# mahfuzalhasan/WaveFormer

Measured on AMD Instinct MI355X. Metric: 128³×4 volumes/sec fwd (1/2/4/8 MI355X) + Dice Δ vs reference, higher is better.
Workload: dtype bf16x3; 1 GPU; MultiscaleTransformer (WaveFormer encoder) forward, 128^3x4 crops; global_batch=8, per_gpu_batch=8, precision=bf16x3, parallelism=replicas x1 (no data-path collective), hip_graph=True

## Files before the change

include/waveformer_hip.h:

```cpp
#ifndef WAVEFORMER_HIP_H
#define WAVEFORMER_HIP_H

#include <stdint.h>

#ifdef __cplusplus
extern "C" {
#endif

#define WF_ABI_VERSION 26

enum { WF_PREC_BF16 = 0, WF_PREC_BF16X3 = 1, WF_PREC_FP16 = 2 };

enum {
  WF_OK = 0,
  WF_E_SHAPE = -1,
  WF_E_NULLPTR = -2,
  WF_E_LAUNCH = -3
};

int wf_abi_version(void);
const char* wf_last_error(void);


int wf_cast_f32_to_bf16(const float* in, uint16_t* out, int64_t n, void* stream);

int wf_split_f32_to_bf16x2(const float* in, uint16_t* out, int64_t n, void* stream);

int wf_split_f32_to_bf16x2_multi(const int64_t* table_dev, int64_t n, int64_t total,
                                 void* stream);

int wf_cast_f32_to_f16x2(const float* in, uint16_t* out, int64_t n, void* stream);
int wf_cast_f32_to_f16x2_multi(const int64_t* table_dev, int64_t n, int64_t total,
                               void* stream);

int wf_debug_poison_lds(int64_t blocks, int lds_bytes, void* stream);

int wf_patch_embed_fwd(const float* x, const float* w, const float* bias, float* out,
                       int64_t B, int64_t Cin, int64_t Cout, int64_t D, int64_t H, int64_t W,
                       void* stream);
int wf_patch_embed_ll_fwd(const float* x, const float* w, const float* bias, float* out,
                          const float* ln_w, const float* ln_b, float ln_eps, float* ll,
                          int64_t B, int64_t Cin, int64_t Cout, int64_t D, int64_t H, int64_t W,
// ... 165 lines not shown
                                        int64_t B, int64_t C, int64_t heads, float scale,
                                        int precision, void* stream, int qkv_mode);
int wf_window_attention_levels_fused(const int64_t* dhw, int nlev, int64_t B, int64_t C,
                                     int64_t heads, int precision);

int wf_msfuse_fwd(const float* const* src, const int64_t* src_dhw, int nsrc,
                  const float* shortcut, const float* branch_scale, float* out, float* stats,
                  float ln_eps, int64_t B, int64_t C, int64_t D, int64_t H, int64_t W,
                  void* stream);

int64_t wf_ccf_ffn_workspace_bytes(int64_t B, int64_t C, int64_t hidden, int64_t D, int64_t H,
                                   int64_t W, int precision);
int wf_ccf_ffn_fwd(const float* xh, const float* stats, const float* n2_w, const float* n2_b,
                   const uint16_t* pw_bf16x2, const float* pw_b, const float* ln1_w,
                   const float* ln1_b, float eps1, const float* dw_w, const float* dw_b,
                   const float* ln2_w, const float* ln2_b, float eps2,
                   const uint16_t* fc_bf16x2, const float* fc_b, const float* branch_scale,
                   float* out, void* workspace,
                   int64_t B, int64_t C, int64_t hidden, int64_t D, int64_t H, int64_t W,
                   int precision, void* stream);
int wf_ccf_ffn_stage(int stage, const float* xh, const float* stats, const float* n2_w,
                     const float* n2_b, const uint16_t* pw_bf16x2, const float* pw_b,
                     const float* ln1_w, const float* ln1_b, float eps1, const float* dw_w,
                     const float* dw_b, const float* ln2_w, const float* ln2_b, float eps2,
                     const uint16_t* fc_bf16x2, const float* fc_b, const float* branch_scale,
                     float* out, void* workspace, int64_t B, int64_t C, int64_t hidden,
                     int64_t D, int64_t H, int64_t W, int precision, void* stream);
int wf_ccf_ffn_plan(int64_t B, int64_t C, int64_t hidden, int64_t D, int64_t H, int64_t W,
                    int precision, int train, int64_t* offsets);

int wf_patch_merging_fwd(const float* x, const float* ln_w, const float* ln_b, float eps,
                         const uint16_t* red_bf16x2, int v2, float* out, int64_t B, int64_t C,
                         int64_t D, int64_t H, int64_t W, int precision, void* stream);

int wf_proj_out_fwd(const float* x, float* out, int normalize, float eps, int64_t B,
                    int64_t C, int64_t S, void* stream);
int wf_proj_out_cl_fwd(const float* x, float* out, float eps, int64_t M, int64_t C, void* stream);

int wf_importance_map(int mode, const float* sigma_scale, float* out, int64_t rd, int64_t rh,
                      int64_t rw, void* stream);

int wf_sliding_window_stitch(const float* patches, int64_t world, int64_t slots_per_round,
                             const float* importance_map, const int64_t* starts,
                             const int64_t* nwin, float* out, int64_t B, int64_t C, int64_t D,
                             int64_t H, int64_t W, int64_t rd, int64_t rh, int64_t rw,
                             void* stream);

int wf_sliding_window_stitch_partial(const float* patches, int64_t world, int64_t rank,
                                     const float* importance_map, const int64_t* starts,
                                     const int64_t* nwin, float* out, int64_t B, int64_t C,
                                     int64_t D, int64_t H, int64_t W, int64_t rd, int64_t rh,
                                     int64_t rw, void* stream);
int wf_sliding_window_normalize(const float* num, float* out, int64_t B, int64_t C, int64_t D,
                                int64_t H, int64_t W, void* stream);

int wf_tta_merge(const float* pred, const int* flips, int npass, float* out, int64_t C,
                 int64_t D, int64_t H, int64_t W, void* stream);


int wf_window_attention_fwd_train(const float* x, const float* ln_w, const float* ln_b,
                                  float ln_eps, const uint16_t* wqkv_bf16x2, const float* bqkv,
                                  const float* bias, const uint16_t* wproj_bf16x2,
                                  const float* bproj, float* out, void* workspace, float* lse,
                                  int64_t B, int64_t C, int64_t D1, int64_t H1, int64_t W1,
                                  int64_t ws, int64_t heads, float scale, int precision,
                                  void* stream);
// ... 144 lines not shown
```

waveformer_amd/_lib.py:

```python
from __future__ import annotations

import ctypes
import os
import threading

_HERE = os.path.dirname(os.path.abspath(__file__))
LIB_PATH = os.environ.get("WAVEFORMER_HIP_LIB", os.path.join(_HERE, "libwaveformer_hip.so"))

_P = ctypes.c_void_p
_I64 = ctypes.c_int64
_I = ctypes.c_int
_F = ctypes.c_float

SIGNATURES = {
    "wf_abi_version": (_I, []),
    "wf_last_error": (ctypes.c_char_p, []),
    "wf_cast_f32_to_bf16": (_I, [_P, _P, _I64, _P]),
    "wf_split_f32_to_bf16x2": (_I, [_P, _P, _I64, _P]),
    "wf_split_f32_to_bf16x2_multi": (_I, [_P, _I64, _I64, _P]),
    "wf_cast_f32_to_f16x2": (_I, [_P, _P, _I64, _P]),
    "wf_cast_f32_to_f16x2_multi": (_I, [_P, _I64, _I64, _P]),
    "wf_debug_poison_lds": (_I, [_I64, _I, _P]),
    "wf_patch_embed_ll_fwd": (_I, [_P, _P, _P, _P, _P, _P, _F, _P, _I64, _I64, _I64, _I64, _I64,
                                   _I64, _P]),
# ... 42 lines not shown
                                _I64, _I64, _I64, _F, _P, _P]),
    "wf_hf_refine_workspace_bytes": (_I64, [_I64, _I64]),
    "wf_hf_refine_fwd": (_I, [_P, _I64, _P, _P, _P, _P, _F, _P, _P, _I, _P, _P, _I64, _I64,
                              _I64, _I64, _I64, _P]),
    "wf_hf_refine_bwd_workspace_bytes": (_I64, [_I64] * 5),
    "wf_hf_refine_bwd": (_I, [_P, _I64, _P, _P, _P, _P, _F, _P, _P, _I, _P, _P, _P, _P, _P, _P,
                              _P, _P, _P, _P, _I64, _I64, _I64, _I64, _I64, _P]),
    "wf_norm_act_cl": (_I, [_P, _I64, _P, _P, _I64, _P, _P, _I64, _I64, _I64, _I64, _F, _P]),
    "wf_upsample_trilinear_cl": (_I, [_P, _P, _I64, _I64, _I64, _I64, _I64, _I64, _I64, _I64,
                                      _I, _P]),
    "wf_linear_fwd": (_I, [_P, _P, _P, _P, _I64, _I64, _I64, _I, _I, _P]),
    "wf_window_attention_fwd_table": (_I, [_P, _P, _P, _F, _P, _P, _P, _P, _P, _P, _P,
                                           _I64, _I64, _I64, _I64, _I64, _I64, _I64, _F, _I,
                                           _P]),
    "wf_rel_pos_bias": (_I, [_P, _P, _P, _I64, _I64, _I64, _P]),
    "wf_window_attention_workspace_bytes": (_I64, [_I64, _I64, _I64, _I64, _I64, _I]),
    "wf_window_attention_fwd": (_I, [_P, _P, _P, _F, _P, _P, _P, _P, _P, _P, _P,
                                     _I64, _I64, _I64, _I64, _I64, _I64, _I64, _F, _I, _P]),
    "wf_window_attention_levels_workspace_bytes": (_I64, [_P, _I, _I64, _I64, _I]),
    "wf_window_attention_fwd_levels": (_I, [_P, _P, _I, _P, _P, _P, _P, _P, _P, _P, _I64, _I64,
                                            _I64, _F, _I, _P]),
    "wf_window_attention_fwd_levels_mode": (_I, [_P, _P, _I, _P, _P, _P, _P, _P, _P, _P, _I64,
                                                 _I64, _I64, _F, _I, _P, _I]),
    "wf_window_attention_levels_fused": (_I, [_P, _I, _I64, _I64, _I64, _I]),
    "wf_msfuse_fwd": (_I, [_P, _P, _I, _P, _P, _P, _P, _F, _I64, _I64, _I64, _I64, _I64, _P]),
    "wf_ccf_ffn_workspace_bytes": (_I64, [_I64, _I64, _I64, _I64, _I64, _I64, _I]),
    "wf_ccf_ffn_fwd": (_I, [_P, _P, _P, _P, _P, _P, _P, _P, _F, _P, _P, _P, _P, _F, _P, _P,
                            _P, _P, _P, _I64, _I64, _I64, _I64, _I64, _I64, _I, _P]),
    "wf_ccf_ffn_stage": (_I, [_I, _P, _P, _P, _P, _P, _P, _P, _P, _F, _P, _P, _P, _P, _F, _P,
                              _P, _P, _P, _P, _I64, _I64, _I64, _I64, _I64, _I64, _I, _P]),
    "wf_ccf_ffn_plan": (_I, [_I64, _I64, _I64, _I64, _I64, _I64, _I, _I, _P]),
    "wf_patch_merging_fwd": (_I, [_P, _P, _P, _F, _P, _I, _P, _I64, _I64, _I64, _I64, _I64,
                                  _I, _P]),
    "wf_proj_out_fwd": (_I, [_P, _P, _I, _F, _I64, _I64, _I64, _P]),
    "wf_proj_out_cl_fwd": (_I, [_P, _P, _F, _I64, _I64, _P]),
    "wf_upsample_dwconv3d_stats_cl": (_I, [_P, _P, _P, _P, _P] + [_I64] * 8 + [_I, _P]),
    "wf_importance_map": (_I, [_I, _P, _P, _I64, _I64, _I64, _P]),
    "wf_sliding_window_stitch": (_I, [_P, _I64, _I64, _P, _P, _P, _P, _I64, _I64, _I64, _I64,
                                      _I64, _I64, _I64, _I64, _P]),
    "wf_tta_merge": (_I, [_P, _P, _I, _P, _I64, _I64, _I64, _I64, _P]),
    "wf_sliding_window_stitch_partial": (_I, [_P, _I64, _I64, _P, _P, _P, _P, _I64, _I64,
                                              _I64, _I64, _I64, _I64, _I64, _I64, _P]),
    "wf_sliding_window_normalize": (_I, [_P, _P, _I64, _I64, _I64, _I64, _I64, _P]),
    "wf_window_attention_fwd_train": (_I, [_P, _P, _P, _F, _P, _P, _P, _P, _P, _P, _P, _P,
                                           _I64, _I64, _I64, _I64, _I64, _I64, _I64, _F, _I,
                                           _P]),
    "wf_window_attention_bwd_workspace_bytes": (_I64, [_I64, _I64, _I64, _I64, _I64, _I64,
                                                       _I64]),
    "wf_window_attention_bwd_core": (_I, [_P, _P, _P, _P, _P, _P, _P, _P, _I64, _I64, _I64,
                                          _I64, _I64, _I64, _I64, _F, _P]),
    "wf_rel_pos_bias_bwd": (_I, [_P, _P, _P, _P, _I64, _I64, _I64, _P]),
    "wf_gemm_tn_workspace_bytes": (_I64, [_I64, _I64, _I64]),
    "wf_gemm_tn": (_I, [_P, _I64, _P, _I64, _P, _I64, _I, _P, _I64, _I64, _I64, _P]),
    "wf_colsum_parts": (_I64, [_I64]),
    "wf_colsum": (_I, [_P, _I64, _I64, _P, _I64, _P, _P, _P]),
    "wf_ln_act_fwd": (_I, [_P, _P, _P, _F, _I, _P, _I64, _I64, _P]),
    "wf_ln_bwd_workspace_floats": (_I64, [_I64, _I64]),
    "wf_ln_act_bwd": (_I, [_P, _P, _P, _F, _I, _P, _P, _P, _P, _P, _P, _I64, _I64, _P]),
    "wf_dwt3d_haar_bwd": (_I, [_P, _P, _P, _I64, _I64, _I64, _I64, _I64, _P]),
    "wf_haar_analysis_ncdhw": (_I, [_P, _I64, _I64, _P, _P, _P, _I64, _I64, _I64, _I64, _I64,
                                    _P]),
    "wf_interp_adjoint_axis": (_I, [_P, _P, _I64, _I64, _I64, _I64, _P, _I64, _P]),
    "wf_interp_adjoint_axis_ac": (_I, [_P, _P, _I64, _I64, _I64, _I64, _P]),
    "wf_dwconv3d_cl": (_I, [_P, _P, _P, _I, _P, _I64, _I64, _I64, _I64, _I64, _P]),
    "wf_dwconv_wgrad_ws_floats": (_I64, [_I64] * 5),
    "wf_dwconv3d_wgrad": (_I, [_P, _P, _P, _P, _I64, _I64, _I64, _I64, _I64, _P]),
    "wf_patch_merging_gather": (_I, [_P, _I, _P, _I64, _I64, _I64, _I64, _I64, _P]),
    "wf_patch_merging_scatter": (_I, [_P, _I, _P, _I64, _I64, _I64, _I64, _I64, _P]),
    "wf_patchify": (_I, [_P, _P, _I, _I64, _I64, _I64, _I64, _I64, _P]),
    "wf_transpose_cs": (_I, [_P, _P, _I64, _I64, _I64, _P]),
    "wf_region_masks": (_I, [_P, _I, _I64, _P, _I64, _P, _P, _P, _I64, _I64, _I64, _P]),
    "wf_overlap_counts": (_I, [_P, _P, _I64, _I64, _I64, _I64, _P, _P]),
    "wf_surface_edt_workspace_bytes": (_I64, [_I64, _I64, _I64, _I64]),
    "wf_surface_edt_sq": (_I, [_P, _I64, _I64, _I64, _I64, _P, _P, _P, _I64, _P]),
    "wf_surface_hist": (_I, [_P, _P, _P, _P, _I64, _I64, _I64, _I64, _P, _P]),
    "wf_hist_order_stats": (_I, [_P, _I64, _I64, _I64, _I64, _I64, _P, _I64, _P, _P]),
    "wf_nonzero_mask": (_I, [_P, _I64, _I64, _I64, _I64, _P, _P]),
    "wf_fill_holes_workspace_bytes": (_I64, [_I64, _I64, _I64]),
    "wf_fill_holes": (_I, [_P, _I64, _I64, _I64, _P, _P, _P, _I64, _P, _P]),
    "wf_box_moments_workspace_bytes": (_I64, [_I64, _I64, _I64, _I64]),
    "wf_box_moments": (_I, [_P, _I64, _I64, _I64, _I64, _P, _P, _P, _I64, _P]),
    "wf_crop_normalize": (_I, [_P, _I64, _I64, _I64, _I64, _P, _P, _P, _P]),
    "wf_crop_seg": (_I, [_P, _P, _I64, _I64, _I64, _P, _I, _P, _P, _P]),
    "wf_select_workspace_bytes": (_I64, [_I64]),
    "wf_select_scan": (_I, [_P, _I64, _I, _I, _P, _I64, _P, _P]),
    "wf_select_pick": (_I, [_P, _I64, _I64, _I64, _I, _I, _P, _I64, _P, _I64, _P, _P, _P, _P]),
    "wf_spline_prefilter_axis": (_I, [_P, _P, _I64, _I64, _I64, _I64, _I, _I, _P]),
    "wf_gauss_blur_axis": (_I, [_P, _P, _I64, _I64, _I64, _I64, _I, _P, _I, _P]),
    "wf_affine_sample": (_I, [_P, _P, _P] + [_I64] * 7 + [_P, _P, _P]),
    "wf_zoom_nearest": (_I, [_P] + [_I64] * 7 + [_P, _P]),
    "wf_zoom_cubic": (_I, [_P] + [_I64] * 7 + [_P, _P]),
    "wf_augment_pointwise_workspace_bytes": (_I64, [_I64, _I64]),
    "wf_augment_pointwise": (_I, [_P, _I64, _I64, _I, _P, _P, _P, _P, _P, _I64, _P]),
    "wf_channel_stats": (_I, [_P, _I64, _I64, _P, _P, _I64, _P]),
}

ABI_VERSION = 26
_lock = threading.Lock()
_lib = None
_err = None


class LibraryMissing(RuntimeError):
    pass


def load(path: str | None = None):
    global _lib, _err
    with _lock:
        if _lib is not None:
            return _lib
        p = path or LIB_PATH
        if not os.path.exists(p):
            _err = f"{p} not found: build it with `python -c 'import __graft_entry__ as g; g.build()'`"
            raise LibraryMissing(_err)
        lib = ctypes.CDLL(p)
        for name, (res, args) in SIGNATURES.items():
            fn = getattr(lib, name)
            fn.restype = res
            fn.argtypes = args
        ver = lib.wf_abi_version()
        if ver != ABI_VERSION:
            raise LibraryMissing(f"{p}: ABI version {ver}, expected {ABI_VERSION} (rebuild)")
        _lib = lib
        return _lib


def call(name: str, *args) -> None:
    lib = load()
    rc = getattr(lib, name)(*args)
# ... 8 lines not shown
```

waveformer_amd/csrc/ffn.hip:

```cpp
#include "kernels.hpp"

namespace wf {

template <typename T>
struct Store4;
template <>
struct Store4<uint16_t> {
  typedef bf16x4 vec;
  static __device__ __forceinline__ f32x4 up(vec u) {
    return f32x4{bf2f((uint16_t)u[0]), bf2f((uint16_t)u[1]), bf2f((uint16_t)u[2]),
                 bf2f((uint16_t)u[3])};
  }
  static __device__ __forceinline__ uint16_t down(float v) { return f2bf(v); }
  static __device__ __forceinline__ vec zero() { return vec{0, 0, 0, 0}; }
  static __device__ __forceinline__ void store4(uint16_t* p, f32x4 v) {
    bf16x4 o;
    o[0] = (short)f2bf(v.x);
    o[1] = (short)f2bf(v.y);
    o[2] = (short)f2bf(v.z);
    o[3] = (short)f2bf(v.w);
    *reinterpret_cast<bf16x4*>(p) = o;
  }
};
template <>
// ... 668 lines not shown
  if (run_dw) {
    if (ln2_loader)
      rc = launch_dwconv3d(h1, dw_w, dw_b, h2, ln2_pst, (int)B, (int)hidden, (int)D, (int)H, (int)W,
                           precision, s, nullptr,
                           plan.front == FFN_FRONT_PARTIALS ? ln1_st : nullptr, ln1_w, ln1_b);
    else
      rc = launch_dwconv_ln_gelu(h1, dw_w, dw_b, ln2_w, ln2_b, eps2, h2, (int)B, (int)hidden,
                                 (int)D, (int)H, (int)W, precision, s);
  }
  if (rc || !run_fc) return rc;
  GemmArgs f = fc_gemm_args(h2, ln2_loader ? ln2_pst : nullptr, ln2_w, ln2_b, eps2, fc_bf16x2, fc_b,
                            xh, stats, n2_w, n2_b, branch_scale, out, M, C, hidden, D * H * W,
                            precision);
  if (!train) {
    f.kpart = reinterpret_cast<float*>(h1);
    f.kpart_bytes = ws.h2 - ws.h1;
  }
  return launch_gemm(f, s, "wf_ccf_ffn_fwd(fc)");
}

extern "C" int wf_ccf_ffn_fwd(const float* xh, const float* stats, const float* n2_w,
                              const float* n2_b, const uint16_t* pw_bf16x2, const float* pw_b,
                              const float* ln1_w, const float* ln1_b, float eps1,
                              const float* dw_w, const float* dw_b, const float* ln2_w,
                              const float* ln2_b, float eps2, const uint16_t* fc_bf16x2,
                              const float* fc_b, const float* branch_scale, float* out,
                              void* workspace, int64_t B, int64_t C, int64_t hidden, int64_t D,
                              int64_t H, int64_t W, int precision, void* stream) {
  return wf_ccf_ffn_stage(0, xh, stats, n2_w, n2_b, pw_bf16x2, pw_b, ln1_w, ln1_b, eps1, dw_w,
                          dw_b, ln2_w, ln2_b, eps2, fc_bf16x2, fc_b, branch_scale, out,
                          workspace, B, C, hidden, D, H, W, precision, stream);
}

extern "C" int wf_patch_merging_fwd(const float* x, const float* ln_w, const float* ln_b,
                                    float eps, const uint16_t* red_bf16x2, int v2, float* out,
                                    int64_t B, int64_t C, int64_t D, int64_t H, int64_t W,
                                    int precision, void* stream) {
  WF_REQUIRE(B >= 1 && C % 8 == 0 && C >= 8, "C must be a positive multiple of 8");
  WF_REQUIRE(D % 2 == 0 && H % 2 == 0 && W % 2 == 0 && D >= 2 && H >= 2 && W >= 2,
             "odd sizes (the F.pad branch, wave_helper.py:180-182) are not supported");
  WF_REQUIRE(valid_prec(precision), "unknown precision");
  WF_REQUIRE_PTR(x);
  WF_REQUIRE_PTR(ln_w);
  WF_REQUIRE_PTR(ln_b);
  WF_REQUIRE_PTR(red_bf16x2);
  WF_REQUIRE_PTR(out);
  GemmArgs g{};
  g.prec = precision;
  g.a_src = x;
  g.a_bf16 = 0;
  g.a_C = (int)C;
  g.a_nseg = 8;
  g.a_map = MAP_MERGE;
  g.merge_code = v2 ? 0x76543210 : 0x71251240;
  g.mB = (int)B;
  g.mD = (int)D;
  g.mH = (int)H;
  g.mW = (int)W;
  g.a_ln = LN_COMPUTE;
  g.a_ln_w = ln_w;
  g.a_ln_b = ln_b;
  g.a_eps = eps;
  g.w = red_bf16x2;
  g.M = B * (D / 2) * (H / 2) * (W / 2);
  g.N = (int)(2 * C);
  g.K = (int)(8 * C);
  g.epi = EPI_STORE;
  g.bias = nullptr;
  g.out = out;
  g.out_bf16 = 0;
  g.ldo = 2 * C;
  if (try_launch_merge_resident(g, (hipStream_t)stream)) return check_launch("wf_patch_merging_fwd");
  return launch_gemm(g, (hipStream_t)stream, "wf_patch_merging_fwd");
}
```

waveformer_amd/csrc/kernels.hpp:

```cpp
#pragma once
#include "ffn_plan.hpp"
#include "wf_common.hpp"

namespace wf {

enum Prec { PREC_BF16 = 0, PREC_SPLIT = 1, PREC_FP16 = 2 };

typedef _Float16 f16x4 __attribute__((ext_vector_type(4)));
typedef _Float16 f16x8 __attribute__((ext_vector_type(8)));
__device__ __forceinline__ uint16_t f2h(float f) { return __builtin_bit_cast(uint16_t, (_Float16)f); }

template <int P>
__device__ __forceinline__ uint16_t op_cvt(float x) {
  if constexpr (P == PREC_FP16) return f2h(x);
  else return f2bf(x);
}
template <int P>
__device__ __forceinline__ short op_lo(float x, uint16_t hi) {
  if constexpr (P == PREC_SPLIT) return (short)f2bf(x - bf2f(hi));
  else return (short)0;
}
template <int P>
__device__ __forceinline__ f32x4 mma32(bf16x8 a, bf16x8 b, f32x4 c) {
  if constexpr (P == PREC_FP16)
    return __builtin_amdgcn_mfma_f32_16x16x32_f16(__builtin_bit_cast(f16x8, a),
                                                  __builtin_bit_cast(f16x8, b), c, 0, 0, 0);
  else return __builtin_amdgcn_mfma_f32_16x16x32_bf16(a, b, c, 0, 0, 0);
}
template <int P>
__device__ __forceinline__ f32x4 mma16(bf16x4 a, bf16x4 b, f32x4 c) {
  if constexpr (P == PREC_FP16)
    return __builtin_amdgcn_mfma_f32_16x16x16f16(__builtin_bit_cast(f16x4, a),
                                                 __builtin_bit_cast(f16x4, b), c, 0, 0, 0);
  else return __builtin_amdgcn_mfma_f32_16x16x16bf16_1k(a, b, c, 0, 0, 0);
// ... 82 lines not shown
  const float* r_scale;
  int64_t rows_per_sample;
  float* o_pstats;
  float* kpart;
  int64_t kpart_bytes;
  int ksplit;
  const float* lv_src[WF_MAX_LEVELS];
  int lv_row0[WF_MAX_LEVELS];
  int lv_D[WF_MAX_LEVELS], lv_H[WF_MAX_LEVELS], lv_W[WF_MAX_LEVELS];
};

int launch_gemm(const GemmArgs& g, hipStream_t s, const char* who);
int gemm_kc_pick_nt(const GemmArgs& g);
int launch_instnorm_partial(const float* x, int64_t ldx, int64_t B, int64_t C, int64_t P,
                            double* acc, hipStream_t s);
int try_launch_gemm_rows(const GemmArgs& g, hipStream_t s, bool single_chunk_only);

int launch_attn_core(const void* qkv, const float* bias, void* out, float* lse, int64_t Bw,
                     int N, int heads, int hd, float scale, int prec, hipStream_t s,
                     int table_ws = 0, int64_t pair_windows = -1, const GemmArgs* fused = nullptr);
bool attn_tbl_pair_loop(int64_t wh);

int launch_dwconv_ln_gelu(const void* in, const float* w, const float* b, const float* ln_w,
                          const float* ln_b, float eps, void* out, int B, int Hd, int D, int H,
                          int W, int prec, hipStream_t s);
int launch_dwconv3d(const void* in, const float* w, const float* b, void* out, float* pstats,
                    int B, int Hd, int D, int H, int W, int prec, hipStream_t s,
                    double* cstats = nullptr, const float* ln1_stats = nullptr,
                    const float* ln1_w = nullptr, const float* ln1_b = nullptr, int flip = 0);
int launch_ln_stats_finalize(const float* pstats, int np, int group, float eps, float* out,
                             int64_t M, hipStream_t s);
int try_launch_gemm_kc(const GemmArgs& g, hipStream_t s);
int try_launch_merge_resident(const GemmArgs& g, hipStream_t s);
int try_launch_pw2_resident(const GemmArgs& g, hipStream_t s);
int try_launch_gemm_lnw(const GemmArgs& g, hipStream_t s);
inline bool gemm_lnw_wide_shape(const GemmArgs& g) { return gemm_lnw_wide_shape(g.N, g.K); }

}

#include "ffn_dwfc_common.hpp"
```

waveformer_amd/csrc/merge.hip:

```cpp
#include <algorithm>

#include "gemm_common.hpp"

namespace wf {

constexpr int MR_C = 48;
constexpr int MR_K = 8 * MR_C;
constexpr int MR_N = 2 * MR_C;
constexpr int MR_NT = MR_N / 16;
constexpr int MR_KS = MR_K / 32;
constexpr int MR_KP = MR_K + WF_LDS_KPAD;
constexpr int MR_WAVES = 8;

template <int P>
__global__ __launch_bounds__(64 * MR_WAVES, 1) void merge_res_kernel(GemmArgs g) {
  constexpr bool SPLIT = P == PREC_SPLIT;
  constexpr int NPL = SPLIT ? 2 : 1;
  extern __shared__ __attribute__((aligned(16))) uint16_t Wl[];
  float* lnw = reinterpret_cast<float*>(Wl + NPL * MR_N * MR_KP);
  float* lnb = lnw + MR_K;
  const int tid = threadIdx.x, lane = tid & 63, wid = tid >> 6;
  const int l15 = lane & 15, g4 = lane >> 4;

  constexpr int OCT = MR_K / 8;
// ... 60 lines not shown
    const float rstd = rsqrtf(fmaxf(q / kf - ms * ms, 0.f) + g.a_eps);

    uint32_t wb = (uint32_t)((l15 * MR_KP + 8 * g4) * 2), lb = (uint32_t)(8 * g4 * 4);
    asm volatile("" : "+v"(wb), "+v"(lb));
    const char* Wb = reinterpret_cast<const char*>(Wl) + wb;
    const char* Lw = reinterpret_cast<const char*>(lnw) + lb;
    const char* Lb = reinterpret_cast<const char*>(lnb) + lb;
    f32x4 acc[MR_NT];
#pragma unroll
    for (int t = 0; t < MR_NT; ++t) acc[t] = f32x4{0.f, 0.f, 0.f, 0.f};
#pragma unroll
    for (int ks = 0; ks < MR_KS; ++ks) {
      __builtin_amdgcn_sched_barrier(0);
      bf16x8 ah, al;
      a_fragment<P>(a[ks], mean, rstd, reinterpret_cast<const float*>(Lw),
                    reinterpret_cast<const float*>(Lb), ks * 32, true, true, false, ah, al);
#pragma unroll
      for (int t = 0; t < MR_NT; ++t) {
        const int wo = (t * 16 * MR_KP + ks * 32) * 2;
        const bf16x8 bh = *reinterpret_cast<const bf16x8*>(Wb + wo);
        const bf16x8 bl = SPLIT ? *reinterpret_cast<const bf16x8*>(Wb + MR_N * MR_KP * 2 + wo) : bh;
        acc[t] = mma3<P>(acc[t], bh, bl, ah, al);
        if (t % 3 == 2) __builtin_amdgcn_sched_barrier(0);
      }
    }
    if (row < M) {
      float* o = reinterpret_cast<float*>(g.out) + (int64_t)row * g.ldo + 4 * g4;
#pragma unroll
      for (int t = 0; t < MR_NT; ++t) *reinterpret_cast<f32x4*>(o + 16 * t) = acc[t];
    }
  }
}

int try_launch_merge_resident(const GemmArgs& g, hipStream_t s) {
  static const bool off = getenv("WF_MERGE_RES") != nullptr && getenv("WF_MERGE_RES")[0] == '0';
  if (off || g.a_map != MAP_MERGE || g.a_C != MR_C || g.K != MR_K || g.N != MR_N ||
      g.a_ln != LN_COMPUTE || g.a_bf16 || g.out_bf16 || g.epi != EPI_STORE || g.bias ||
      g.o_pstats || g.ldo < MR_N || (g.prec != PREC_SPLIT && g.prec != PREC_FP16) || g.M < 1 ||
      g.M >= ((int64_t)1 << 31) - 16)
    return 0;
  const bool split = g.prec == PREC_SPLIT;
  const size_t lds = (size_t)(split ? 2 : 1) * MR_N * MR_KP * 2 + (size_t)2 * MR_K * 4;
  void (*kern)(GemmArgs) = split ? merge_res_kernel<PREC_SPLIT> : merge_res_kernel<PREC_FP16>;
  set_max_lds(reinterpret_cast<const void*>(kern), (int)lds);
  const int64_t ntiles = (g.M + 15) / 16;
  const unsigned gx = (unsigned)std::min<int64_t>(cdiv(ntiles, MR_WAVES), 256);
  hipLaunchKernelGGL(kern, dim3(gx), dim3(64 * MR_WAVES), lds, s, g);
  return 1;
}

}
```

waveformer_amd/network_models/wave_helper.py:

```python
from __future__ import annotations

import math
import threading
from typing import Optional, Tuple

import torch
import torch.nn as nn
import torch.nn.functional as F

from .. import autograd as wfa
from .. import library
from .. import ops
from .attention import Attention

_OPS = torch.ops.waveformer


def _conv_fan_out_init(m: nn.Module) -> None:
    if isinstance(m, (nn.Conv2d, nn.Conv3d)):
        fan_out = math.prod(m.kernel_size) * m.out_channels // m.groups
        m.weight.data.normal_(0, math.sqrt(2.0 / fan_out))
        if m.bias is not None:
            m.bias.data.zero_()

# ... 138 lines not shown
        return y.flatten(2).transpose(1, 2)


class PatchMergingV2(nn.Module):

    def __init__(self, dim: int, norm_layer=nn.LayerNorm, spatial_dims: int = 3) -> None:
        super().__init__()
        self.dim = dim
        if spatial_dims == 3:
            self.reduction = nn.Linear(8 * dim, 2 * dim, bias=False)
            self.norm = norm_layer(8 * dim)
        elif spatial_dims == 2:
            self.reduction = nn.Linear(4 * dim, 2 * dim, bias=False)
            self.norm = norm_layer(4 * dim)
        self._v2 = True

    def _merge_2d(self, x):
        b, h, w, c = x.shape
        if h % 2 or w % 2:
            x = F.pad(x, (0, 0, 0, w % 2, 0, h % 2))
        x = torch.cat([x[:, j::2, i::2, :] for i in range(2) for j in range(2)], -1)
        return self.reduction(self.norm(x))

    def forward(self, x):
        if x.dim() == 4:
            return self._merge_2d(x)
        if x.dim() != 5:
            raise ValueError(f"expecting 5D x, got {tuple(x.shape)}.")
        b, d, h, w, c = x.shape
        if d % 2 or h % 2 or w % 2:
            x = F.pad(x, (0, 0, 0, w % 2, 0, h % 2, 0, d % 2))
        x = x.contiguous()
        prec = wfa.prec_for(x, *self.parameters())
        return _OPS.patch_merging(x, self.norm.weight, self.norm.bias, float(self.norm.eps),
                                  self.reduction.weight, self._v2, prec)

    def _wf_split_params(self):
        return [self.reduction.weight]


class PatchMerging(PatchMergingV2):

    def __init__(self, dim: int, norm_layer=nn.LayerNorm, spatial_dims: int = 3) -> None:
        super().__init__(dim, norm_layer, spatial_dims)
        self._v2 = False


class CCF_FFN(nn.Module):

    def __init__(self, in_features, hidden_features=None, out_features=None,
                 act_layer=nn.GELU, norm_layer=nn.LayerNorm, drop=0., img_size=(48, 48, 48)):
        super().__init__()
        self.D, self.H, self.W = img_size[0], img_size[1], img_size[2]
        out_features = out_features or in_features
        hidden_features = hidden_features or in_features
        self.C_hid = hidden_features
        self.pwconv = nn.Conv3d(in_features, hidden_features, 1, 1, 0, bias=True)
        self.dwconv = nn.Conv3d(hidden_features, hidden_features, 3, 1, 1, bias=True,
                                groups=hidden_features)
        self.fc = nn.Linear(hidden_features, in_features)
        self.act = act_layer()
        self.norm1 = norm_layer(hidden_features)
        self.norm2 = norm_layer(hidden_features)
        if not (isinstance(self.act, nn.GELU) and self.act.approximate == "none"):
            raise NotImplementedError("CCF_FFN: only nn.GELU() (erf) is implemented")
        self.apply(self._init_weights)

    def _init_weights(self, m):
# ... 292 lines not shown
```

waveformer_amd/ops.py:

```python
from __future__ import annotations

import ctypes
import math
import os
import threading
import weakref
from typing import Dict, List, Optional, Sequence, Tuple

import torch

from . import _lib

DETAIL_KEYS = ("aad", "ada", "add", "daa", "dad", "dda", "ddd")


def _stream() -> int:
    return torch.cuda.current_stream().cuda_stream


def _ptr(t: Optional[torch.Tensor]) -> Optional[int]:
    return None if t is None else t.data_ptr()


def _check(t: torch.Tensor, name: str, dtype=torch.float32, contiguous=True) -> None:
# ... 1308 lines not shown
    fc = split_weight(fcw, prec=prec)
    out = torch.empty_like(xh)
    wsb = _lib.query("wf_ccf_ffn_workspace_bytes", B, C, hid, D, H, W, prec)
    work = torch.empty(wsb, dtype=torch.uint8, device=xh.device)
    args = (xh.data_ptr(), _ptr(stats), _ptr(n2w), _ptr(n2b),
            pw.data_ptr(), _ptr(pwb), l1w.data_ptr(), l1b.data_ptr(), float(eps1),
            dww.data_ptr(), dwb.data_ptr(), l2w.data_ptr(), l2b.data_ptr(), float(eps2),
            fc.data_ptr(), _ptr(fcb), _ptr(branch_scale),
            out.data_ptr(), work.data_ptr(), B, C, hid, D, H, W, prec, _stream())
    ccf_ffn_pwconv(args)
    ccf_ffn_dwconv(args, B * D * H * W, hid)
    ccf_ffn_fc(args)
    return out


def ccf_ffn_pwconv(args):
    _lib.call("wf_ccf_ffn_stage", 1, *args)


def ccf_ffn_dwconv(args, positions: int, hidden: int):
    _lib.call("wf_ccf_ffn_stage", 2, *args)


def ccf_ffn_fc(args):
    _lib.call("wf_ccf_ffn_stage", 3, *args)


def patch_merging(x_cl: torch.Tensor, norm: torch.nn.LayerNorm, reduction: torch.nn.Linear,
                  v2: bool = False) -> torch.Tensor:
    return _patch_merging_raw(x_cl, norm.weight, norm.bias, float(norm.eps), reduction.weight,
                              v2, _prec())


def _patch_merging_raw(x_cl, ln_w, ln_b, eps, red_w, v2, prec) -> torch.Tensor:
    _check(x_cl, "x")
    B, D, H, W, C = x_cl.shape
    red = split_weight(red_w, prec=prec)
    out = torch.empty((B, D // 2, H // 2, W // 2, 2 * C), dtype=torch.float32, device=x_cl.device)
    _lib.call("wf_patch_merging_fwd", x_cl.data_ptr(), ln_w.data_ptr(), ln_b.data_ptr(),
              float(eps), red.data_ptr(), int(bool(v2)), out.data_ptr(), B, C, D, H, W, prec,
              _stream())
    return out


BLEND_MODES = {"constant": 0, "gaussian": 1}


def importance_map(roi: Sequence[int], mode: str = "constant",
                   sigma_scale: Sequence[float] = (0.125, 0.125, 0.125),
                   device: Optional[torch.device] = None) -> torch.Tensor:
    if mode not in BLEND_MODES:
        raise ValueError(f"Unsupported mode: {mode}, available options are {sorted(BLEND_MODES)}.")
    rd, rh, rw = (int(v) for v in roi)
    device = torch.device(device) if device is not None else torch.device(
        "cuda", torch.cuda.current_device())
    if device.type != "cuda":
        raise RuntimeError("importance_map: GPU only")
    out = torch.empty((rd, rh, rw), dtype=torch.float32, device=device)
    sig = (ctypes.c_float * 3)(*[float(s) for s in sigma_scale])
    _lib.call("wf_importance_map", BLEND_MODES[mode], sig, out.data_ptr(), rd, rh, rw, _stream())
    return out


def sliding_window_stitch(patches: torch.Tensor, weight_map: torch.Tensor,
                          starts: Sequence[Sequence[int]], image_size: Sequence[int],
                          batch: int, world: int = 1, slots_per_round: int = 1) -> torch.Tensor:
    _check(patches, "patches")
    _check(weight_map, "importance_map")
    rows, C = patches.shape[:2]
    roi = tuple(patches.shape[2:])
    if tuple(weight_map.shape) != roi:
        raise ValueError(f"sliding_window_stitch: map {tuple(weight_map.shape)} != roi {roi}")
    nwin = [len(s) for s in starts]
    total = batch * nwin[0] * nwin[1] * nwin[2]
# ... 536 lines not shown
```

Baseline: 1317 volumes/s.

## Add persistent streaming patch-merging kernel with fused LayerNorm for C=96/192

Adds a persistent, register-streamed patch-merge kernel for C=96 and C=192 at inference. Each block loops over row tiles, gathers the 2x2x2 neighbours into LDS, computes LayerNorm there and runs the bf16x3 or fp16 MFMA GEMM. Weights are pre-permuted into a workspace so each wave streams its own slice through a triple-buffered register pipeline, and C=96 adds dedicated loader waves to prefetch the next tile. The aim is to replace the generic GEMM path for these merges. The cost is an extra weight-permute launch per call and a per-call workspace allocation.

```diff
diff --git a/include/waveformer_hip.h b/include/waveformer_hip.h
--- a/include/waveformer_hip.h
+++ b/include/waveformer_hip.h
@@ -7,7 +7,7 @@
 extern "C" {
 #endif
 
-#define WF_ABI_VERSION 26
+#define WF_ABI_VERSION 27
 
 enum { WF_PREC_BF16 = 0, WF_PREC_BF16X3 = 1, WF_PREC_FP16 = 2 };
 
@@ -239,6 +239,13 @@
 int wf_patch_merging_fwd(const float* x, const float* ln_w, const float* ln_b, float eps,
                          const uint16_t* red_bf16x2, int v2, float* out, int64_t B, int64_t C,
                          int64_t D, int64_t H, int64_t W, int precision, void* stream);
+int64_t wf_patch_merging_workspace_bytes(int64_t C, int precision);
+int wf_patch_merging_fwd_ws(const float* x, const float* ln_w, const float* ln_b, float eps,
+                            const uint16_t* red_bf16x2, int v2, float* out, int64_t B, int64_t C,
+                            int64_t D, int64_t H, int64_t W, int precision, int train,
+                            void* workspace, int64_t workspace_bytes, void* stream);
+int wf_patch_merging_plan(int64_t B, int64_t C, int64_t D, int64_t H, int64_t W, int precision,
+                          int train, int64_t* info);
 
 int wf_proj_out_fwd(const float* x, float* out, int normalize, float eps, int64_t B,
                     int64_t C, int64_t S, void* stream);
diff --git a/waveformer_amd/_lib.py b/waveformer_amd/_lib.py
--- a/waveformer_amd/_lib.py
+++ b/waveformer_amd/_lib.py
@@ -98,6 +98,10 @@
     "wf_ccf_ffn_plan": (_I, [_I64, _I64, _I64, _I64, _I64, _I64, _I, _I, _P]),
     "wf_patch_merging_fwd": (_I, [_P, _P, _P, _F, _P, _I, _P, _I64, _I64, _I64, _I64, _I64,
                                   _I, _P]),
+    "wf_patch_merging_workspace_bytes": (_I64, [_I64, _I]),
+    "wf_patch_merging_fwd_ws": (_I, [_P, _P, _P, _F, _P, _I, _P, _I64, _I64, _I64, _I64, _I64,
+                                     _I, _I, _P, _I64, _P]),
+    "wf_patch_merging_plan": (_I, [_I64, _I64, _I64, _I64, _I64, _I, _I, _P]),
     "wf_proj_out_fwd": (_I, [_P, _P, _I, _F, _I64, _I64, _I64, _P]),
     "wf_proj_out_cl_fwd": (_I, [_P, _P, _F, _I64, _I64, _P]),
     "wf_upsample_dwconv3d_stats_cl": (_I, [_P, _P, _P, _P, _P] + [_I64] * 8 + [_I, _P]),
@@ -161,7 +165,7 @@
     "wf_channel_stats": (_I, [_P, _I64, _I64, _P, _P, _I64, _P]),
 }
 
-ABI_VERSION = 26
+ABI_VERSION = 27
 _lock = threading.Lock()
 _lib = None
 _err = None
diff --git a/waveformer_amd/csrc/ffn.hip b/waveformer_amd/csrc/ffn.hip
--- a/waveformer_amd/csrc/ffn.hip
+++ b/waveformer_amd/csrc/ffn.hip
@@ -724,10 +724,28 @@
                           workspace, B, C, hidden, D, H, W, precision, stream);
 }
 
-extern "C" int wf_patch_merging_fwd(const float* x, const float* ln_w, const float* ln_b,
-                                    float eps, const uint16_t* red_bf16x2, int v2, float* out,
-                                    int64_t B, int64_t C, int64_t D, int64_t H, int64_t W,
-                                    int precision, void* stream) {
+extern "C" int64_t wf_patch_merging_workspace_bytes(int64_t C, int precision) {
+  return merge_stream_bytes(C, precision);
+}
+
+extern "C" int wf_patch_merging_plan(int64_t B, int64_t C, int64_t D, int64_t H, int64_t W,
+                                     int precision, int train, int64_t* info) {
+  WF_REQUIRE(B >= 1 && C >= 8 && D >= 2 && H >= 2 && W >= 2, "empty shape");
+  WF_REQUIRE(valid_prec(precision), "unknown precision");
+  WF_REQUIRE_PTR(info);
+  const int kind = merge_plan(B, C, D, H, W, precision, train != 0, merge_res_off());
+  const int64_t M = B * (D / 2) * (H / 2) * (W / 2);
+  info[0] = kind;
+  info[1] = kind == MERGE_STREAM ? merge_stream_mr(C) : 0;
+  info[2] = kind == MERGE_STREAM ? merge_stream_passes(M, C) : 0;
+  info[3] = kind == MERGE_STREAM ? merge_stream_blocks(M, C) : 0;
+  return 0;
+}
+
+static int patch_merging_fwd(const float* x, const float* ln_w, const float* ln_b, float eps,
+                             const uint16_t* red_bf16x2, int v2, float* out, int64_t B, int64_t C,
+                             int64_t D, int64_t H, int64_t W, int precision, int train,
+                             void* workspace, int64_t workspace_bytes, void* stream) {
   WF_REQUIRE(B >= 1 && C % 8 == 0 && C >= 8, "C must be a positive multiple of 8");
   WF_REQUIRE(D % 2 == 0 && H % 2 == 0 && W % 2 == 0 && D >= 2 && H >= 2 && W >= 2,
              "odd sizes (the F.pad branch, wave_helper.py:180-182) are not supported");
@@ -762,6 +780,27 @@
   g.out = out;
   g.out_bf16 = 0;
   g.ldo = 2 * C;
-  if (try_launch_merge_resident(g, (hipStream_t)stream)) return check_launch("wf_patch_merging_fwd");
+  const int rc = try_launch_merge_stream(g, train != 0, workspace, workspace_bytes, (hipStream_t)stream);
+  if (rc < 0) return rc;
+  if (rc || try_launch_merge_resident(g, (hipStream_t)stream)) return check_launch("wf_patch_merging_fwd");
   return launch_gemm(g, (hipStream_t)stream, "wf_patch_merging_fwd");
 }
+
+extern "C" int wf_patch_merging_fwd(const float* x, const float* ln_w, const float* ln_b,
+                                    float eps, const uint16_t* red_bf16x2, int v2, float* out,
+                                    int64_t B, int64_t C, int64_t D, int64_t H, int64_t W,
+                                    int precision, void* stream) {
+  return patch_merging_fwd(x, ln_w, ln_b, eps, red_bf16x2, v2, out, B, C, D, H, W, precision, 0,
+                           nullptr, 0, stream);
+}
+
+extern "C" int wf_patch_merging_fwd_ws(const float* x, const float* ln_w, const float* ln_b,
+                                       float eps, const uint16_t* red_bf16x2, int v2, float* out,
+                                       int64_t B, int64_t C, int64_t D, int64_t H, int64_t W,
+                                       int precision, int train, void* workspace,
+                                       int64_t workspace_bytes, void* stream) {
+  WF_REQUIRE(workspace_bytes >= 0 && (workspace != nullptr || workspace_bytes == 0),
+             "workspace_bytes without a workspace");
+  return patch_merging_fwd(x, ln_w, ln_b, eps, red_bf16x2, v2, out, B, C, D, H, W, precision,
+                           train, workspace, workspace_bytes, stream);
+}
diff --git a/waveformer_amd/csrc/kernels.hpp b/waveformer_amd/csrc/kernels.hpp
--- a/waveformer_amd/csrc/kernels.hpp
+++ b/waveformer_amd/csrc/kernels.hpp
@@ -1,5 +1,6 @@
 #pragma once
 #include "ffn_plan.hpp"
+#include "merge_plan.hpp"
 #include "wf_common.hpp"
 
 namespace wf {
@@ -148,6 +149,9 @@
                              int64_t M, hipStream_t s);
 int try_launch_gemm_kc(const GemmArgs& g, hipStream_t s);
 int try_launch_merge_resident(const GemmArgs& g, hipStream_t s);
+int try_launch_merge_stream(const GemmArgs& g, bool train, void* workspace, int64_t workspace_bytes,
+                            hipStream_t s);
+bool merge_res_off();
 int try_launch_pw2_resident(const GemmArgs& g, hipStream_t s);
 int try_launch_gemm_lnw(const GemmArgs& g, hipStream_t s);
 inline bool gemm_lnw_wide_shape(const GemmArgs& g) { return gemm_lnw_wide_shape(g.N, g.K); }
diff --git a/waveformer_amd/csrc/merge.hip b/waveformer_amd/csrc/merge.hip
--- a/waveformer_amd/csrc/merge.hip
+++ b/waveformer_amd/csrc/merge.hip
@@ -116,9 +116,13 @@
   }
 }
 
+bool merge_res_off() {
+  static const bool off = getenv("WF_MERGE_RES") != nullptr && getenv("WF_MERGE_RES")[0] == '0';
+  return off;
+}
+
 int try_launch_merge_resident(const GemmArgs& g, hipStream_t s) {
-  static const bool off = getenv("WF_MERGE_RES") != nullptr && getenv("WF_MERGE_RES")[0] == '0';
-  if (off || g.a_map != MAP_MERGE || g.a_C != MR_C || g.K != MR_K || g.N != MR_N ||
+  if (merge_res_off() || g.a_map != MAP_MERGE || g.a_C != MR_C || g.K != MR_K || g.N != MR_N ||
       g.a_ln != LN_COMPUTE || g.a_bf16 || g.out_bf16 || g.epi != EPI_STORE || g.bias ||
       g.o_pstats || g.ldo < MR_N || (g.prec != PREC_SPLIT && g.prec != PREC_FP16) || g.M < 1 ||
       g.M >= ((int64_t)1 << 31) - 16)
@@ -133,4 +137,257 @@
   return 1;
 }
 
-}
+template <int CIN>
+struct MsCfg {
+  static constexpr int K = 8 * CIN, N = 2 * CIN, KS = K / 32;
+  static constexpr int MR = merge_stream_mr(CIN), RT = MR / 16;
+  static constexpr int WAVES = merge_stream_waves(CIN), LW = merge_stream_loaders(CIN);
+  static constexpr int WALL = WAVES + LW, NTHR = 64 * WALL;
+  static constexpr int LT = LW ? 64 * LW : NTHR;
+  static constexpr int RS = K + 8;
+  static constexpr int TPR = LT / MR;
+  static constexpr int QPT = (K / 4) / TPR;
+  static constexpr int OPL = (K / 8 + 63) / 64;
+  static constexpr size_t LDS = (size_t)(MR * RS + 2 * K + 2 * MR) * 4;
+  static_assert(N == 16 * MERGE_NTW * WAVES && KS % 3 == 0 && (K / 4) % TPR == 0 && MR % 16 == 0, "shape");
+  static_assert(LDS <= 160 * 1024, "LDS");
+};
+
+template <int NPL>
+__global__ __launch_bounds__(256) void merge_wstream_kernel(const uint16_t* __restrict__ w,
+                                                             uint16_t* __restrict__ out, int N, int K) {
+  const int i = blockIdx.x * 256 + threadIdx.x;
+  if (i >= NPL * N * (K / 8)) return;
+  const int KS = K / 32;
+  const int lane = i & 63;
+  int r = i >> 6;
+  const int pl = r % NPL;
+  r /= NPL;
+  const int t = r % MERGE_NTW;
+  r /= MERGE_NTW;
+  const int ks = r % KS, wave = r / KS;
+  const int l15 = lane & 15, g4 = lane >> 4;
+  const uint16_t* src = w + (size_t)pl * N * K + (size_t)(wave * (16 * MERGE_NTW) + 16 * t + l15) * K + ks * 32 + 8 * g4;
+  *reinterpret_cast<bf16x8*>(out + (size_t)i * 8) = *reinterpret_cast<const bf16x8*>(src);
+}
+
+template <int P, int CIN>
+__global__ __launch_bounds__(64 * (merge_stream_waves(CIN) + merge_stream_loaders(CIN)), 1) void merge_stream_kernel(
+    GemmArgs g, const uint16_t* __restrict__ wst) {
+  typedef MsCfg<CIN> C;
+  constexpr bool SPLIT = P == PREC_SPLIT;
+  constexpr int NPL = SPLIT ? 2 : 1, NTW = MERGE_NTW, NR = 3;
+  constexpr int K = C::K, KS = C::KS, MR = C::MR, RT = C::RT, RS = C::RS;
+  extern __shared__ __attribute__((aligned(16))) float At[];
+  float* lnw = At + MR * RS;
+  float* lnb = lnw + K;
+  float* st = lnb + K;
+  const int tid = threadIdx.x, lane = tid & 63;
+  const int wid = __builtin_amdgcn_readfirstlane(tid >> 6);
+  const int l15 = lane & 15, g4 = lane >> 4;
+  for (int i = tid; i < K; i += C::NTHR) {
+    lnw[i] = g.a_ln_w[i];
+    lnb[i] = g.a_ln_b[i];
+  }
+  const int M = (int)g.M;
+  const int passes = (M + MR - 1) / MR;
+
+  const __amdgpu_buffer_rsrc_t wrsrc = buf_rsrc(wst, NPL * C::N * K * 2);
+  const int wvoff = (wid % C::WAVES) * (KS * NTW * NPL * 1024) + 16 * lane;
+  const bf16x8 z8 = {0, 0, 0, 0, 0, 0, 0, 0};
+  bf16x8 wh[NR][NTW], wl[NR][NTW];
+  auto wload = [&](int ks, auto slot) {
+    constexpr int SL = decltype(slot)::value;
+    const int k = ks >= KS ? ks - KS : ks;
+#pragma unroll
+    for (int t = 0; t < NTW; ++t) {
+      const int so = (k * NTW + t) * NPL * 1024;
+      wh[SL][t] = __builtin_bit_cast(bf16x8, __builtin_amdgcn_raw_buffer_load_b128(wrsrc, wvoff, so, 0));
+      wl[SL][t] = SPLIT ? __builtin_bit_cast(bf16x8, __builtin_amdgcn_raw_buffer_load_b128(
+                                                         wrsrc, wvoff, so + 1024, 0))
+                        : z8;
+    }
+  };
+  typedef std::integral_constant<int, 0> I0;
+  typedef std::integral_constant<int, 1> I1;
+  typedef std::integral_constant<int, 2> I2;
+  if (wid < C::WAVES) {
+    wload(0, I0());
+    wload(1, I1());
+  }
+
+  auto bar = [&]() {
+    asm volatile("s_waitcnt lgkmcnt(0)" ::: "memory");
+    __builtin_amdgcn_s_barrier();
+    asm volatile("" ::: "memory");
+  };
+  constexpr bool PF = C::LW > 0;
+  const bool loader = PF ? wid >= C::WAVES : true;
+  const int ltid = PF ? tid - 64 * C::WAVES : tid;
+  const int grow = ltid / C::TPR, gu = ltid % C::TPR;
+  const float* src = reinterpret_cast<const float*>(g.a_src);
+  f32x4 gv[C::QPT];
+  auto gload = [&](int p) {
+    const RowMapper<MAP_MERGE> rm(g, min(p * MR + grow, M - 1));
+#pragma unroll
+    for (int j = 0; j < C::QPT; ++j) {
+      const int k = 4 * (gu + C::TPR * j);
+      const int seg = k / CIN, c = k - seg * CIN;
+      const int o = (g.merge_code >> (4 * seg)) & 0xF;
+      const int pp = rm.pos + (((o >> 2) & 1) * g.mH + ((o >> 1) & 1)) * g.mW + (o & 1);
+      gv[j] = *reinterpret_cast<const f32x4*>(src + (int64_t)pp * CIN + c);
+    }
+  };
+  auto gstore = [&]() {
+#pragma unroll
+    for (int j = 0; j < C::QPT; ++j)
+      *reinterpret_cast<f32x4*>(At + grow * RS + 4 * (gu + C::TPR * j)) = gv[j];
+  };
+  if (PF && loader && (int)blockIdx.x < passes) gload(blockIdx.x);
+  __syncthreads();
+  for (int p = blockIdx.x; p < passes; p += gridDim.x) {
+    const int r0 = p * MR;
+    bar();
+    if (loader) {
+      if (!PF) gload(p);
+      gstore();
+    }
+    bar();
+    if (PF && loader && p + (int)gridDim.x < passes) gload(p + gridDim.x);
+    if (wid < RT) {
+      const int row = 16 * wid + l15;
+      const float* rp = At + row * RS;
+      const float sh = rp[0];
+      float s = 0.f, q = 0.f;
+#pragma unroll 4
+      for (int i = 0; i < KS; ++i) {
+        const f32x4 a = *reinterpret_cast<const f32x4*>(rp + 8 * (g4 + 4 * i));
+        const f32x4 b = *reinterpret_cast<const f32x4*>(rp + 8 * (g4 + 4 * i) + 4);
+        const float x[8] = {a.x, a.y, a.z, a.w, b.x, b.y, b.z, b.w};
+#pragma unroll
+        for (int j = 0; j < 8; ++j) {
+          const float d = x[j] - sh;
+          s += d;
+          q = __builtin_fmaf(d, d, q);
+        }
+      }
+      s = xsum16(s);
+      s = xsum32(s);
+      q = xsum16(q);
+      q = xsum32(q);
+      const float kf = (float)g.K;
+      const float ms = s / kf;
+      const float mean = sh + ms;
+      const float rstd = rsqrtf(fmaxf(q / kf - ms * ms, 0.f) + g.a_eps);
+      if (g4 == 0) {
+        st[2 * row] = mean;
+        st[2 * row + 1] = rstd;
+      }
+    }
+    bar();
+    for (int r = wid; r < MR; r += C::WALL) {
+      float* rp = At + r * RS;
+      const float mean = st[2 * r], rstd = st[2 * r + 1];
+      float v[C::OPL][8];
+#pragma unroll
+      for (int j = 0; j < C::OPL; ++j) {
+        const int o = min(lane + 64 * j, K / 8 - 1);
+        const f32x4 a = *reinterpret_cast<const f32x4*>(rp + 8 * o);
+        const f32x4 b = *reinterpret_cast<const f32x4*>(rp + 8 * o + 4);
+        v[j][0] = a.x; v[j][1] = a.y; v[j][2] = a.z; v[j][3] = a.w;
+        v[j][4] = b.x; v[j][5] = b.y; v[j][6] = b.z; v[j][7] = b.w;
+      }
+      asm volatile("s_waitcnt lgkmcnt(0)" ::: "memory");
+      __builtin_amdgcn_sched_barrier(0);
+      uint16_t* rb = reinterpret_cast<uint16_t*>(rp);
+#pragma unroll
+      for (int j = 0; j < C::OPL; ++j) {
+        const int o = lane + 64 * j;
+        bf16x8 ah, al;
+        a_fragment<P>(v[j], mean, rstd, lnw, lnb, 8 * min(o, K / 8 - 1), true, true, false, ah, al);
+        if (o < K / 8) {
+          *reinterpret_cast<bf16x8*>(rb + 8 * o) = ah;
+          if (SPLIT) *reinterpret_cast<bf16x8*>(rb + K + 8 * o) = al;
+        }
+      }
+    }
+    bar();
+    if (PF && loader) continue;
+    f32x4 acc[RT][NTW];
+#pragma unroll
+    for (int rt = 0; rt < RT; ++rt)
+#pragma unroll
+      for (int t = 0; t < NTW; ++t) acc[rt][t] = f32x4{0.f, 0.f, 0.f, 0.f};
+    const uint16_t* Ab = reinterpret_cast<const uint16_t*>(At) + l15 * (2 * RS) + 8 * g4;
+    bf16x8 ah[RT], al[RT];
+    auto aload = [&](int ks) {
+#pragma unroll
+      for (int rt = 0; rt < RT; ++rt) {
+        const uint16_t* q = Ab + rt * 16 * (2 * RS) + ks * 32;
+        ah[rt] = *reinterpret_cast<const bf16x8*>(q);
+        al[rt] = SPLIT ? *reinterpret_cast<const bf16x8*>(q + K) : z8;
+      }
+    };
+    auto kstep = [&](int ks, auto slot) {
+      constexpr int SL = decltype(slot)::value;
+      wload(ks + 2, std::integral_constant<int, (SL + 2) % NR>());
+      __builtin_amdgcn_sched_barrier(0);
+#pragma unroll
+      for (int t = 0; t < NTW; ++t)
+#pragma unroll
+        for (int rt = 0; rt < RT; ++rt)
+          acc[rt][t] = mma3<P>(acc[rt][t], wh[SL][t], wl[SL][t], ah[rt], al[rt]);
+      __builtin_amdgcn_sched_barrier(0);
+      aload(min(ks + 1, KS - 1));
+    };
+    aload(0);
+#pragma unroll 1
+    for (int ks = 0; ks < KS; ks += NR) {
+      kstep(ks, I0());
+      kstep(ks + 1, I1());
+      kstep(ks + 2, I2());
+    }
+#pragma unroll
+    for (int rt = 0; rt < RT; ++rt) {
+      const int row = r0 + 16 * rt + l15;
+      if (row < M) {
+        float* o = reinterpret_cast<float*>(g.out) + (int64_t)row * g.ldo + 16 * NTW * wid + 4 * g4;
+#pragma unroll
+        for (int t = 0; t < NTW; ++t) *reinterpret_cast<f32x4*>(o + 16 * t) = acc[rt][t];
+      }
+    }
+  }
+}
+
+template <int CIN>
+static void go_merge_stream(const GemmArgs& g, uint16_t* wst, hipStream_t s) {
+  typedef MsCfg<CIN> C;
+  const bool split = g.prec == PREC_SPLIT;
+  const int nfrag = (split ? 2 : 1) * C::N * (C::K / 8);
+  if (split)
+    hipLaunchKernelGGL(merge_wstream_kernel<2>, dim3(cdiv(nfrag, 256)), dim3(256), 0, s, g.w, wst, C::N, C::K);
+  else
+    hipLaunchKernelGGL(merge_wstream_kernel<1>, dim3(cdiv(nfrag, 256)), dim3(256), 0, s, g.w, wst, C::N, C::K);
+  void (*kern)(GemmArgs, const uint16_t*) =
+      split ? merge_stream_kernel<PREC_SPLIT, CIN> : merge_stream_kernel<PREC_FP16, CIN>;
+  set_max_lds(reinterpret_cast<const void*>(kern), (int)C::LDS);
+  const unsigned gx = (unsigned)merge_stream_blocks(g.M, CIN);
+  hipLaunchKernelGGL(kern, dim3(gx), dim3(C::NTHR), C::LDS, s, g, (const uint16_t*)wst);
+}
+
+int try_launch_merge_stream(const GemmArgs& g, bool train, void* workspace, int64_t workspace_bytes,
+                            hipStream_t s) {
+  if (g.a_map != MAP_MERGE || g.a_ln != LN_COMPUTE || g.a_bf16 || g.out_bf16 || g.epi != EPI_STORE ||
+      g.bias || g.o_pstats || g.K != 8 * g.a_C || g.N != 2 * g.a_C || g.ldo != g.N)
+    return 0;
+  if (merge_plan(g.mB, g.a_C, g.mD, g.mH, g.mW, g.prec, train, merge_res_off()) != MERGE_STREAM)
+    return 0;
+  if (!workspace) return 0;
+  if (workspace_bytes < merge_stream_bytes(g.a_C, g.prec))
+    return fail(WF_E_SHAPE, "wf_patch_merging_fwd_ws: workspace smaller than wf_patch_merging_workspace_bytes");
+  if (g.a_C == 96) go_merge_stream<96>(g, reinterpret_cast<uint16_t*>(workspace), s);
+  else go_merge_stream<192>(g, reinterpret_cast<uint16_t*>(workspace), s);
+  return 1;
+}
+
+}
diff --git a/waveformer_amd/csrc/merge_plan.hpp b/waveformer_amd/csrc/merge_plan.hpp
--- /dev/null
+++ b/waveformer_amd/csrc/merge_plan.hpp
@@ -0,0 +1,57 @@
+#pragma once
+#include <stdint.h>
+
+namespace wf {
+
+constexpr int kMergePrecBf16 = 0;
+constexpr bool merge_store32(int prec) { return prec != kMergePrecBf16; }
+
+enum MergeKernel {
+  MERGE_GEMM_KC = 0,
+  MERGE_RESIDENT = 1,
+  MERGE_STREAM = 2,
+};
+
+constexpr int MERGE_NTW = 3;
+constexpr int MERGE_CUS = 256;
+constexpr bool merge_stream_cin(int64_t C) { return C == 96 || C == 192; }
+constexpr int merge_stream_mr(int64_t C) { return C == 96 ? 32 : 16; }
+constexpr int merge_stream_waves(int64_t C) { return (int)(2 * C / (16 * MERGE_NTW)); }
+constexpr int merge_stream_loaders(int64_t C) { return C == 96 ? 4 : 0; }
+inline int64_t merge_stream_passes(int64_t M, int64_t C) {
+  const int mr = merge_stream_mr(C);
+  return (M + mr - 1) / mr;
+}
+inline int64_t merge_stream_blocks(int64_t M, int64_t C) {
+  const int64_t p = merge_stream_passes(M, C);
+  return p < MERGE_CUS ? p : MERGE_CUS;
+}
+inline int64_t merge_stream_bytes(int64_t C, int prec) {
+  return merge_stream_cin(C) && merge_store32(prec) ? 2 * (2 * C) * (8 * C) * 2 : 0;
+}
+
+inline int64_t merge_stream_index(int npl, int64_t K, int pl, int64_t n, int64_t k) {
+  const int64_t ksteps = K / 32;
+  const int64_t wave = n / (16 * MERGE_NTW), t = (n / 16) % MERGE_NTW, l15 = n % 16;
+  const int64_t ks = k / 32, g4 = (k % 32) / 8, j = k % 8;
+  const int64_t lane = 16 * g4 + l15;
+  return (((((wave * ksteps + ks) * MERGE_NTW + t) * npl + pl) * 64) + lane) * 8 + j;
+}
+inline int64_t merge_stream_step_elems(int npl) { return (int64_t)MERGE_NTW * npl * 64 * 8; }
+inline int64_t merge_stream_step_base(int npl, int64_t K, int64_t wave, int64_t ks) {
+  return (wave * (K / 32) + ks) * merge_stream_step_elems(npl);
+}
+
+inline int merge_plan(int64_t B, int64_t C, int64_t D, int64_t H, int64_t W, int prec, bool train,
+                      bool merge_res_off) {
+  if (merge_res_off || !merge_store32(prec)) return MERGE_GEMM_KC;
+  if (C == 48) return MERGE_RESIDENT;
+  if (!merge_stream_cin(C) || train) return MERGE_GEMM_KC;
+  const int64_t M = B * (D / 2) * (H / 2) * (W / 2);
+  if (M < 1) return MERGE_GEMM_KC;
+  const int64_t lim = (int64_t)1 << 31;
+  if (B * D * H * W * C * 4 >= lim || M * 2 * C * 4 >= lim) return MERGE_GEMM_KC;
+  return MERGE_STREAM;
+}
+
+}
diff --git a/waveformer_amd/network_models/wave_helper.py b/waveformer_amd/network_models/wave_helper.py
--- a/waveformer_amd/network_models/wave_helper.py
+++ b/waveformer_amd/network_models/wave_helper.py
@@ -194,8 +194,11 @@
             x = F.pad(x, (0, 0, 0, w % 2, 0, h % 2, 0, d % 2))
         x = x.contiguous()
         prec = wfa.prec_for(x, *self.parameters())
-        return _OPS.patch_merging(x, self.norm.weight, self.norm.bias, float(self.norm.eps),
-                                  self.reduction.weight, self._v2, prec)
+        train = torch.is_grad_enabled() and (
+            x.requires_grad or any(p.requires_grad for p in self.parameters()))
+        with ops.merge_training(train):
+            return _OPS.patch_merging(x, self.norm.weight, self.norm.bias, float(self.norm.eps),
+                                      self.reduction.weight, self._v2, prec)
 
     def _wf_split_params(self):
         return [self.reduction.weight]
diff --git a/waveformer_amd/ops.py b/waveformer_amd/ops.py
--- a/waveformer_amd/ops.py
+++ b/waveformer_amd/ops.py
@@ -1364,14 +1364,35 @@
                               v2, _prec())
 
 
+_merge_tls = threading.local()
+
+
+class merge_training:
+
+    def __init__(self, flag: bool):
+        self.flag = bool(flag)
+
+    def __enter__(self):
+        self.prev = getattr(_merge_tls, "train", False)
+        _merge_tls.train = self.flag
+        return self
+
+    def __exit__(self, *exc):
+        _merge_tls.train = self.prev
+        return False
+
+
 def _patch_merging_raw(x_cl, ln_w, ln_b, eps, red_w, v2, prec) -> torch.Tensor:
     _check(x_cl, "x")
     B, D, H, W, C = x_cl.shape
     red = split_weight(red_w, prec=prec)
     out = torch.empty((B, D // 2, H // 2, W // 2, 2 * C), dtype=torch.float32, device=x_cl.device)
-    _lib.call("wf_patch_merging_fwd", x_cl.data_ptr(), ln_w.data_ptr(), ln_b.data_ptr(),
+    train = bool(getattr(_merge_tls, "train", False))
+    wsb = 0 if train else _lib.query("wf_patch_merging_workspace_bytes", C, prec)
+    ws = torch.empty(wsb, dtype=torch.uint8, device=x_cl.device) if wsb > 0 else None
+    _lib.call("wf_patch_merging_fwd_ws", x_cl.data_ptr(), ln_w.data_ptr(), ln_b.data_ptr(),
               float(eps), red.data_ptr(), int(bool(v2)), out.data_ptr(), B, C, D, H, W, prec,
-              _stream())
+              int(train), ws.data_ptr() if ws is not None else None, wsb, _stream())
     return out
 
 
```

Result: no change. 1328 volumes/s (median of 6 runs) (+0.8%).
